# christoskokas/gtsam-vSLAM

Hardware: AMD Instinct MI355X
Metric: frames/sec (extract+match+localBA), 1500 feat stereo 752x480 (higher is better)
Workload: dtype u8/i32 (extract, match) + f64 (pose LM, local BA)

## Files before the change

gtsam-vslam_amd/csrc/ba.hip:

```cpp
#include "common.hpp"
#include "comm.hpp"
#include "dmath.hpp"
#include "ba_pool.hpp"
#include "ba_packed.hpp"
#include "ba_types.hpp"
#include "ba_order_host.hpp"
#include "ba_plan.hpp"
#include <algorithm>
#include <cmath>
#include <vector>

namespace vslam {

static_assert(BA_MAX_LEVELS == MAX_LEVELS, "BaChi::thr holds one threshold per pyramid level");
__device__ __forceinline__ int ba_slot(int sel, int c, int NB) {
    const int s = sel + 1 + c;
    return s > NB ? s - (NB + 1) : s;
}
__device__ __forceinline__ bool ba_enter(BaDev& D, int state, int c = 0) {
    const int* ci = (const int*)(D.ctl + CTL_INTS);
    if (ci[CI_STATE] != state) return false;
    D.nAct = ci[CI_NACT];
    if (c >= D.nAct) return false;
    const int sel = ci[CI_SEL], ts = ba_slot(sel, c, D.NB);
// ... 478 lines not shown
        __syncthreads();
        for (int k = 0; k < nc; k++) {
            double* dst = SpartBase + (size_t)(c0 + k) * D.spartStride + (size_t)blockIdx.x * sys;
            for (int i = threadIdx.x; i < (int)sys; i += nt) dst[i] = Sloc[(size_t)k * sys + i];
        }
    }
}

__device__ __forceinline__ double ba2_dpp_xor(double v, int which) {
    const int lo = __double2loint(v), hi = __double2hiint(v);
    int l2, h2;
    if (which == 0) { l2 = __builtin_amdgcn_update_dpp(0, lo, 0xB1, 0xF, 0xF, true); h2 = __builtin_amdgcn_update_dpp(0, hi, 0xB1, 0xF, 0xF, true); }
    else { l2 = __builtin_amdgcn_update_dpp(0, lo, 0x4E, 0xF, 0xF, true); h2 = __builtin_amdgcn_update_dpp(0, hi, 0x4E, 0xF, 0xF, true); }
    return __hiloint2double(h2, l2);
}
struct Ba2Roles {
    int hk, hq, hx, hy, hyStep; bool hOn; double hSign;
    int ws, wi;
    __device__ __forceinline__ void init(int lane) {
        hk = lane >> 2; hq = lane & 3; hOn = hk < 9;
        const int ha = hk < 3 ? 0 : (hk < 5 ? 1 : (hk == 5 ? 2 : hk - 6));
        const int hbx = hk < 3 ? hk : (hk < 5 ? hk - 2 : 2);
        hx = 14 + ha;
        hy = hk < 6 ? 14 + hbx : 0;
        hyStep = hk < 6 ? 3 : 1;
        hSign = hk < 6 ? 1.0 : -1.0;
        ws = lane / 6; wi = lane - ws * 6;
    }
};
struct Ba2Region { double* F; double* W; double* WH; double* hb; int* ffi; int* sst; int* sfi; };
__device__ __forceinline__ Ba2Region ba2_region(double* base, int maxFac, int maxSlots) {
    Ba2Region g;
    g.F = base; g.W = g.F + maxFac * 20; g.WH = g.W + maxSlots * 18; g.hb = g.WH + maxSlots * 18;
    g.ffi = (int*)(g.hb + 10); g.sst = g.ffi + maxFac; g.sfi = g.sst + maxSlots + 1;
    return g;
}
__device__ __forceinline__ void ba2_stage_h(const BaDev& D, int lp, const Ba2Region& g, const Ba2Roles& R, int lane, double* h, int& nf, int& ns) {
    const int f0 = D.lpStart[lp], s0 = D.lpSlotStart[lp];
    nf = D.lpStart[lp + 1] - f0;
    ns = D.lpSlotStart[lp + 1] - s0 - 1;
    {
        const double2* src = (const double2*)(D.facJ + (size_t)f0 * 20);
        double2* dst = (double2*)g.F;
        for (int i = lane; i < nf * 10; i += 64) dst[i] = src[i];
        for (int i = lane; i < nf; i += 64) g.ffi[i] = D.facFi[f0 + i];
        for (int i = lane; i <= ns; i += 64) { g.sst[i] = D.slotStart[s0 + i] - f0; g.sfi[i] = D.slotFi[s0 + i]; }
    }
    ba_wave_fence();
    {
        double acc = 0;
        if (R.hOn)
            for (int f = R.hq; f < nf; f += 4) {
                const double* o = g.F + f * 20;
                acc += o[R.hx] * o[R.hy] + o[R.hx + 3] * o[R.hy + R.hyStep];
            }
        acc += ba2_dpp_xor(acc, 0);
        acc += ba2_dpp_xor(acc, 1);
        if (R.hOn && R.hq == 0) g.hb[R.hk] = R.hSign * acc;
    }
    ba_wave_fence();
#pragma unroll
    for (int k = 0; k < 9; k++) h[k] = g.hb[k];
}
__device__ __forceinline__ void ba2_w_row(const Ba2Region& g, const Ba2Roles& R, double& w0, double& w1, double& w2) {
    w0 = w1 = w2 = 0;
    for (int f = g.sst[R.ws]; f < g.sst[R.ws + 1]; f++) {
        const double* o = g.F + f * 20;
        const double a0 = o[2 + R.wi], a1 = o[8 + R.wi];
        w0 += a0 * o[14] + a1 * o[17];
        w1 += a0 * o[15] + a1 * o[18];
        w2 += a0 * o[16] + a1 * o[19];
    }
}

template <bool PACKED>
__device__ __forceinline__ void ba2_blocks(double* Sloc, const double* W, const double* WH, const int* sfi, int ns, int lane, int F, int ld) {
    const int nb = ns * (ns + 1) / 2, half = lane & 1;
    for (int b0 = 0; b0 < nb; b0 += 32) {
        int b = b0 + (lane >> 1), s1 = 0;
        if (b >= nb) continue;
        while (b >= ns - s1) { b -= ns - s1; s1++; }
        const int s2 = s1 + b;
        const double* A = WH + s1 * 18 + half * 9;
        const double* B = W + s2 * 18;
        double aa[9];
#pragma unroll
        for (int q = 0; q < 9; q++) aa[q] = A[q];
        double* d0 = Sloc + (PACKED ? ba_packed_block(F, sfi[s1], sfi[s2]) * BA_PACKED_PITCH + 18 * half : (6 * sfi[s1] + 3 * half) * ld + 6 * sfi[s2]);
#pragma unroll
        for (int jh = 0; jh < 2; jh++) {
            double bb[9];
#pragma unroll
            for (int q = 0; q < 9; q++) bb[q] = B[9 * jh + q];
#pragma unroll
            for (int i = 0; i < 3; i++) {
                double* dr = d0 + i * (PACKED ? 6 : ld) + 3 * jh;
#pragma unroll
                for (int j = 0; j < 3; j++) atomicAdd(dr + j, -(aa[3 * i] * bb[3 * j] + aa[3 * i + 1] * bb[3 * j + 1] + aa[3 * i + 2] * bb[3 * j + 2]));
            }
        }
    }
}

template <bool PACKED>
__device__ __forceinline__ void ba2_schur(const BaDev* __restrict__ tab, int maxSlots, int maxFac, int layout) {
    BaDev D = *lane_entry(tab, blockIdx.z);
    extern __shared__ double sm[];
    if (!ba_enter(D, BA_TRY, blockIdx.y)) return;
    const int n = D.n, F = n / 6;
    constexpr bool packed = PACKED;
    const int ld = layout == BA2_ROWMAJOR1 ? n + 1 : n;
    const int sys = ba2_sys_doubles(n, layout);
    double* const Sloc = sm;
    double* const racc = Sloc + (packed ? ba_packed_rhs(F) : ld * n);
    const int lane = threadIdx.x & 63;
    const int unit = __builtin_amdgcn_readfirstlane(threadIdx.x >> 6), nu = blockDim.x >> 6, nt = blockDim.x;
    const Ba2Region g = ba2_region(sm + sys + (size_t)unit * ba2_stage_doubles(maxFac, maxSlots), maxFac, maxSlots);
    double* const F_ = g.F; double* const W = g.W; double* const WH = g.WH;
    int* const ffi = g.ffi; int* const sfi = g.sfi;
    const double lam = D.lambda;
    Ba2Roles R;
    R.init(lane);
    const int pf = lane / 6, pi = lane - pf * 6;
    for (int i = threadIdx.x; i < sys; i += nt) Sloc[i] = 0;
    __syncthreads();
    for (int lp = blockIdx.x * nu + unit; lp < D.Lp; lp += gridDim.x * nu) {
        double h[9];
        int nf, ns;
        ba2_stage_h(D, lp, g, R, lane, h, nf, ns);
        double Hi[9];
        ba_hll_inverse(h, lam, Hi);
        if (R.ws < ns) {
            double w0, w1, w2;
            ba2_w_row(g, R, w0, w1, w2);
            const double g0 = w0 * Hi[0] + w1 * Hi[3] + w2 * Hi[6], g1 = w0 * Hi[1] + w1 * Hi[4] + w2 * Hi[7], g2 = w0 * Hi[2] + w1 * Hi[5] + w2 * Hi[8];
            double* wr = W + R.ws * 18 + R.wi * 3;
            wr[0] = w0; wr[1] = w1; wr[2] = w2;
            double* gr = WH + R.ws * 18 + R.wi * 3;
            gr[0] = g0; gr[1] = g1; gr[2] = g2;
            atomicAdd(&racc[6 * sfi[R.ws] + R.wi], -(g0 * h[6] + g1 * h[7] + g2 * h[8]));
        }
        ba_wave_fence();
        ba2_blocks<PACKED>(Sloc, W, WH, sfi, ns, lane, F, ld);
        if (pf < 10)
            for (int fb = 0; fb < nf; fb += 10) {
                const int f = fb + pf;
                if (f >= nf) break;
                const int fi = ffi[f];
                if (fi < 0) continue;
                const double* o = F_ + f * 20;
                const double a0 = o[2 + pi], a1 = o[8 + pi];
                double* dr = Sloc + (packed ? ba_packed_block(F, fi, fi) * BA_PACKED_PITCH + 6 * pi : (6 * fi + pi) * ld + 6 * fi);
                for (int j = pi; j < 6; j++) atomicAdd(dr + j, a0 * o[2 + j] + a1 * o[8 + j]);
                atomicAdd(&racc[6 * fi + pi], -(a0 * o[0] + a1 * o[1]));
            }
        ba_wave_fence();
    }
    __syncthreads();
    const int part = ba2_part_doubles(n, layout);
    double* dst = D.Spart + (size_t)blockIdx.x * part;
    if (layout == BA2_ROWMAJOR1) {
        for (int i = threadIdx.x; i < part; i += nt) dst[i] = Sloc[i + i / n];
    } else {
        for (int i = threadIdx.x; i < part; i += nt) dst[i] = Sloc[i];
    }
}
__global__ __launch_bounds__(1024) void k_ba_schur2(const BaDev* __restrict__ tab, int maxSlots, int maxFac) { ba2_schur<true>(tab, maxSlots, maxFac, BA2_PACKED); }
__global__ __launch_bounds__(1024) void k_ba_schur2_rm(const BaDev* __restrict__ tab, int maxSlots, int maxFac, int layout) { ba2_schur<false>(tab, maxSlots, maxFac, layout); }

__global__ __launch_bounds__(512) void k_ba_back2(const BaDev* __restrict__ tab, int maxSlots, int maxFac) {
    BaDev D = *lane_entry(tab, blockIdx.z);
    extern __shared__ double sm[];
    if (!ba_enter(D, BA_TRY, 0)) return;
    const int nc = D.nAct;
    const int sel = ((const int*)(D.ctl + CTL_INTS))[CI_SEL];
    const int lane = threadIdx.x & 63;
    const int unit = __builtin_amdgcn_readfirstlane(threadIdx.x >> 6), nu = blockDim.x >> 6;
    const Ba2Region g = ba2_region(sm + (size_t)unit * ba2_stage_doubles(maxFac, maxSlots), maxFac, maxSlots);
    Ba2Roles R;
    R.init(lane);
    for (int lp = blockIdx.x * nu + unit; lp < D.Lp; lp += gridDim.x * nu) {
        double h[9];
        int nf, ns;
        ba2_stage_h(D, lp, g, R, lane, h, nf, ns);
        double w0 = 0, w1 = 0, w2 = 0;
        int kcol = 0;
        if (R.ws < ns) { ba2_w_row(g, R, w0, w1, w2); kcol = 6 * g.sfi[R.ws] + R.wi; }
        const int l = D.lpOrig[lp];
        double lamk = D.lambda;
        for (int k = 0; k < nc; k++, lamk *= 10.0) {
            const double* dPk = D.dP + (size_t)k * D.n;
            const double dp = R.ws < ns ? dPk[kcol] : 0.0;
            double t0 = w0 * dp, t1 = w1 * dp, t2 = w2 * dp;
            t0 += ba2_dpp_xor(t0, 0); t1 += ba2_dpp_xor(t1, 0); t2 += ba2_dpp_xor(t2, 0);
            t0 += ba2_dpp_xor(t0, 1); t1 += ba2_dpp_xor(t1, 1); t2 += ba2_dpp_xor(t2, 1);
#pragma unroll
            for (int d = 4; d <= 32; d <<= 1) { t0 += __shfl_xor(t0, d); t1 += __shfl_xor(t1, d); t2 += __shfl_xor(t2, d); }
            double Hi[9];
            ba_hll_inverse(h, lamk, Hi);
            if (lane < 3) {
                const double u0 = h[6] - t0, u1 = h[7] - t1, u2 = h[8] - t2;
                const double h0 = lane == 0 ? Hi[0] : (lane == 1 ? Hi[3] : Hi[6]);
                const double h1 = lane == 0 ? Hi[1] : (lane == 1 ? Hi[4] : Hi[7]);
                const double h2 = lane == 0 ? Hi[2] : (lane == 1 ? Hi[5] : Hi[8]);
                const double dl = h0 * u0 + h1 * u1 + h2 * u2;
                D.dL[(size_t)k * D.dLStride + 3 * (size_t)lp + lane] = dl;
                double* lmT = D.lmBase + (size_t)ba_slot(sel, k, D.NB) * D.lmStride;
                lmT[3 * (size_t)l + lane] = D.lmCur[3 * (size_t)l + lane] + dl;
            }
        }
        ba_wave_fence();
    }
}

__global__ __launch_bounds__(256) void k_ba_reduce(const BaDev* __restrict__ tab, int nPart, int packed) {
    BaDev D = *lane_entry(tab, blockIdx.z);
    __shared__ double sSl[8][33];
    if (!ba_enter(D, BA_TRY, blockIdx.y)) return;
    const int total = D.n * D.n + D.n, F = D.n / 6;
    const int nSum = packed ? ba_packed_doubles(F) : total;
    const int nSlots = packed ? ba_packed_reduce_slots(F) : total;
    const int e = threadIdx.x & 31, y = threadIdx.x >> 5;
    const int i = blockIdx.x * 32 + e;
    double s = 0;
    if (i < nSum) {
        const int per = (nPart + 7) / 8;
// ... 1984 lines not shown
            }
        }
    }
    BHS("chi2");
    BHS("fetch");
    if (!resultFetched) {
        VS_HIP(hipMemcpyAsync(poseOut, poseFinal, K * sizeof(DPose), hipMemcpyDeviceToHost, stream));
        if (L) VS_HIP(hipMemcpyAsync(lmOut, lmFinal, (size_t)3 * L * sizeof(double), hipMemcpyDeviceToHost, stream));
        VS_HIP(hipStreamSynchronize(stream));
    }
    ba_write_result(R, poseOut, lmOut, wrong.data(), K, L, NP);
    return VSLAM_OK;
}

static std::atomic<long long> g_bbsNs[12], g_bbsCalls{0}, g_bbsPolls{0};
static const char* g_bbsName[12] = {"check+count", "arena fill", "tables+upload", "lm pass 1", "chi2 1", "second-pass prep", "lm pass 2", "chi2 2 + fetch", "results", nullptr, nullptr, nullptr};

static BaPlanKnobs ba_plan_knobs() {
    static const bool s2Env = !(getenv("VSLAM_BA_SCHUR2") && atoi(getenv("VSLAM_BA_SCHUR2")) == 0);
    static const bool b2Env = !(getenv("VSLAM_BA_BACK2") && atoi(getenv("VSLAM_BA_BACK2")) == 0);
    BaPlanKnobs k;
    k.schur2 = s2Env; k.back2 = b2Env;
    k.sharedW = getenv("VSLAM_BA_SCHUR_SHARED") ? atoi(getenv("VSLAM_BA_SCHUR_SHARED")) != 0 : true;
    k.schurWaves = getenv("VSLAM_BA_SCHUR_WAVES_B") ? atoi(getenv("VSLAM_BA_SCHUR_WAVES_B")) : 0;
    k.lmBlocks = getenv("VSLAM_BA_LMBLOCKS") ? atoi(getenv("VSLAM_BA_LMBLOCKS")) : 0;
    k.s2Waves = getenv("VSLAM_BA_SCHUR2_WAVES") ? atoi(getenv("VSLAM_BA_SCHUR2_WAVES")) : 8;
    k.b2Waves = getenv("VSLAM_BA_BACK2_WAVES") ? atoi(getenv("VSLAM_BA_BACK2_WAVES")) : 4;
    k.s2Layout = getenv("VSLAM_BA_SCHUR2_LAYOUT") ? std::max(0, std::min((int)BA2_PACKED, atoi(getenv("VSLAM_BA_SCHUR2_LAYOUT")))) : (int)BA2_PACKED;
    return k;
}
thread_local vslam_ba_batch_plan g_baLastPlan{};

static vslam_status ba_run_batch(const vslam_ba_problem* const* Ps, vslam_ba_result* const* Rs, int N, int device) {
    g_baLastPlan = vslam_ba_batch_plan{};
    if (N <= 0 || !Ps || !Rs) return VSLAM_ERR_INVALID;
    if (N == 1) { g_baLastPlan.n_single = 1; return ba_run(Ps[0], Rs[0], device, nullptr); }
    auto bbs_t = std::chrono::steady_clock::now();
    g_bbsCalls++;
    auto BBS = [&](int k) { const auto t_ = std::chrono::steady_clock::now(); g_bbsNs[k] += std::chrono::duration_cast<std::chrono::nanoseconds>(t_ - bbs_t).count(); bbs_t = t_; };
    VS_CHECK(ba_select_device(device));
    struct BatchWs {
        hipStream_t stream = nullptr; int device = -1;
        PinnedArena arena;
// ... 123 lines not shown
        const Lane& q = lanes[i];
        nMax = std::max(nMax, q.H.n); neMax = std::max(neMax, q.H.NE);
        nfMax = std::max(nfMax, q.H.NF); npMax = std::max(npMax, q.NP);
        valMax = std::max(valMax, std::max(q.K * (int)(sizeof(DPose) / sizeof(double)), 3 * q.L));
    }
    plan_cohort();
    const vslam_ba_batch_plan& plan = g_baLastPlan;
    if (plan.status != VSLAM_OK) { set_error("local BA batch: landmark with too many views for the LDS staging"); return VSLAM_ERR_CAPACITY; }
    const int nCU = BA_NCU;
    const int obsBlocks = std::max(1, std::min((nfMax + 255) / 256, std::max(16, 2 * nCU / NL)));
    const int facBlocks = obsBlocks + std::max(neMax, 1);
    const size_t sysMax = (size_t)nMax * nMax + nMax;
    const int maxSlots = plan.max_slots, maxFac = plan.max_factors, lmBlocks = plan.schur_blocks;
    const bool useSchur2 = plan.schur_kernel == VSLAM_BA_KERNEL_SCHUR2, useBack2 = plan.back_kernel == VSLAM_BA_KERNEL_BACK2;
    const int s2Layout = ba_plan_knobs().s2Layout;
    const bool packedS = useSchur2 && s2Layout == BA2_PACKED;
    const int reduceSlots = packedS ? ba_packed_reduce_slots(nMax / 6) : (int)sysMax;
    auto part_doubles = [&](int n) { return (size_t)(useSchur2 ? ba2_part_doubles(n, s2Layout) : n * n + n); };
    const bool anyMfma64 = plan.solve_kinds & (1 << BA_SOLVE_MFMA64), anyWave = plan.solve_kinds & (1 << BA_SOLVE_WAVE),
               anyMfma = plan.solve_kinds & (1 << BA_SOLVE_MFMA);
    VS_CHECK(ba_kernel_attributes());
    size_t dBytes = 0;
    auto dtake = [&](size_t bytes) { const size_t at = dBytes; dBytes = (dBytes + std::max<size_t>(bytes, 8) + 255) & ~(size_t)255; return at; };
    struct Off { size_t flags, sedge, poseS, lmS, facJ, dP, dL, S, partial, spart, sums, Lg, wrong, outPose, outLm; };
    std::vector<Off> off(NL);
    for (int a = 0; a < NL; a++) { const Lane& q = lanes[act[a]]; off[a].flags = dtake(16 * sizeof(int)); off[a].sedge = dtake(((size_t)q.H.n * q.H.n + q.H.n) * nSlots * 8); }
    const size_t zeroBytes = dBytes;
    size_t wrongBase = 0, wrongEnd = 0, outBase = 0, outEnd = 0;
    wrongBase = dBytes;
    for (int a = 0; a < NL; a++) off[a].wrong = dtake(lanes[act[a]].NP);
    wrongEnd = dBytes;
// ... 51 lines not shown
    const BaDev* const dTab = A.dev(h_tab);
    const BaLaneAux* const dAux = A.dev(h_aux);
    VS_HIP(A.upload(stream));
    VS_HIP(hipMemsetAsync(dm, 0, zeroBytes, stream));
    const int valBlocks = std::max(1, std::min((valMax + 255) / 256, 64));
    hipLaunchKernelGGL(k_ba_init_slots_b, dim3(valBlocks, NL), dim3(256), 0, stream, dTab, dAux);

    auto step = [&](bool first) -> vslam_status {
        int t = -1;
        if (first) {
            t = g_baTimer.begin("ba_linearize");
            hipLaunchKernelGGL(k_ba_factors<0>, dim3(facBlocks, 1, NL), dim3(256), 0, stream, dTab, obsBlocks, 1, relTol, absTol);
            g_baTimer.end(t);
        }
        t = g_baTimer.begin("ba_schur");
        if (useSchur2 && s2Layout == BA2_PACKED) hipLaunchKernelGGL(k_ba_schur2, dim3(lmBlocks, NB, NL), dim3(64 * plan.schur_waves), plan.schur_lds, stream, dTab, maxSlots, maxFac);
        else if (useSchur2) hipLaunchKernelGGL(k_ba_schur2_rm, dim3(lmBlocks, NB, NL), dim3(64 * plan.schur_waves), plan.schur_lds, stream, dTab, maxSlots, maxFac, s2Layout);
        else hipLaunchKernelGGL(k_ba_schur, dim3(lmBlocks, plan.schur_shared_w ? 1 : NB, NL), dim3(64 * plan.schur_waves), plan.schur_lds, stream, dTab, maxSlots, plan.schur_shared_w);
        g_baTimer.end(t);
        t = g_baTimer.begin("ba_solve");
        hipLaunchKernelGGL(k_ba_reduce, dim3((reduceSlots + 31) / 32, NB, NL), dim3(256), 0, stream, dTab, lmBlocks, packedS ? 1 : 0);
        if (anyMfma64) hipLaunchKernelGGL(k_ba_solve_mfma64, dim3(NB, 1, NL), dim3(64), 0, stream, dTab);
        if (anyWave) hipLaunchKernelGGL(k_ba_solve_wave, dim3(NB, 1, NL), dim3(64), 0, stream, dTab);
        if (anyMfma) hipLaunchKernelGGL(k_ba_solve_mfma, dim3(NB, 1, NL), dim3(64 * BA_MFMA_NW), plan.solve_lds, stream, dTab, (double*)nullptr);
        g_baTimer.end(t);
        t = g_baTimer.begin("ba_back");
        if (useBack2) hipLaunchKernelGGL(k_ba_back2, dim3(plan.back_blocks, 1, NL), dim3(64 * plan.back_waves), plan.back_lds, stream, dTab, maxSlots, maxFac);
        else hipLaunchKernelGGL(k_ba_back, dim3(plan.back_blocks, plan.back_shared ? 1 : NB, NL), dim3(64 * plan.back_waves), plan.back_lds, stream, dTab, maxSlots, plan.back_shared);
        g_baTimer.end(t);
        t = g_baTimer.begin("ba_eval");
        hipLaunchKernelGGL(k_ba_factors<1>, dim3(facBlocks, NB, NL), dim3(256), 0, stream, dTab, obsBlocks, 1, relTol, absTol);
        g_baTimer.end(t);
        VS_HIP(hipGetLastError());
        return VSLAM_OK;
    };
    double* const b_ctl = (double*)(W.h_back + oBackCtl);
    memcpy(b_ctl, h_ctlAll, (size_t)CTL_DOUBLES * 8 * NL);
    auto lm_loop = [&](int first) -> vslam_status {
        static const int perPollEnv = getenv("VSLAM_BA_STEPS_PER_POLL") ? std::max(1, atoi(getenv("VSLAM_BA_STEPS_PER_POLL"))) : 0;
        int enq = 0, polls = 0;
        for (;;) {
            const int batch = perPollEnv ? perPollEnv : (enq == 0 ? first : 2);
// ... 82 lines not shown
        const double* lo = (const double*)(W.h_back + q.oOut + (((size_t)q.K * sizeof(DPose) + 255) & ~(size_t)255));
        ba_write_result(q.R, po, lo, W.h_back + q.oWrong, q.K, q.L, q.NP);
    }
    BBS(8);
    for (int i : redo) VS_CHECK(ba_run(Ps[i], Rs[i], device, nullptr));
    return run_singles();
}

namespace vslam {
void ba_host_profile_print() {
#ifndef VSLAM_HOST_STAMPS
    if (const long long nb = g_bbsCalls.load()) {
        fprintf(stderr, "  vslam_local_ba_batch host sections (us per cohort, %lld cohorts, %.1f polls each):", nb, (double)g_bbsPolls.load() / (double)nb);
        for (int i = 0; i < 12 && g_bbsName[i]; i++) fprintf(stderr, " %s %.1f |", g_bbsName[i], 1e-3 * (double)g_bbsNs[i].load() / (double)nb);
        fprintf(stderr, "\n");
    }
    const long long n = g_bhsCalls.load();
    if (!n) return;
    fprintf(stderr, "  vslam_local_ba host sections (us per call, %lld calls):", n);
    for (int i = 0; i < 16; i++) if (g_bhsName[i] || g_bhsNs[i].load()) fprintf(stderr, " %s %.1f |", g_bhsName[i] ? g_bhsName[i] : "other", 1e-3 * (double)g_bhsNs[i].load() / (double)n);
    fprintf(stderr, "\n");
#endif
}
}

extern "C" {

vslam_status vslam_local_ba(const vslam_ba_problem* problem, vslam_ba_result* result, int32_t device,
                            const vslam_comm* comm) {
    return ba_run(problem, result, device, comm);
// ... 211 lines not shown
```

gtsam-vslam_amd/csrc/ba_plan.hpp:

```cpp
#pragma once
#include "ba_types.hpp"
#include "ba_order_host.hpp"
#include <initializer_list>

namespace vslam {

constexpr int BA_NCU = 256;
constexpr size_t BA_LDS_SOFT = 150 * 1024;
constexpr int BA_SCHUR_LPW = 64 / BA_LPL_SCHUR, BA_BACK_LPW = 64 / BA_LPL_BACK;
inline size_t ba_stage_lds(int nw, int maxSlots) { return (size_t)nw * BA_SCHUR_LPW * 2 * maxSlots * 18 * sizeof(double) + (size_t)nw * BA_SCHUR_LPW * maxSlots * sizeof(int) + 16; }
inline size_t ba_schur_lds(int nw, int copies, size_t sysDoubles, int maxSlots) { return copies * sysDoubles * sizeof(double) + ba_stage_lds(nw, maxSlots); }
inline size_t ba_back_lds(int nw, int maxSlots) { return (size_t)nw * BA_BACK_LPW * maxSlots * 18 * sizeof(double) + (size_t)nw * BA_BACK_LPW * maxSlots * sizeof(int) + 16; }
inline int ba_schur_waves(int NB, bool allowShared, int cap, int start, size_t sysDoubles, int maxSlots, int& sharedW) {
    sharedW = 0;
    if (NB > 1 && allowShared)
        for (int nw : {16, 12, 8, 6, 4, 2})
            if (nw <= cap && ba_schur_lds(nw, NB, sysDoubles, maxSlots) <= BA_LDS_SOFT) { sharedW = 1; return nw; }
    while (start > 2 && ba_schur_lds(start, 1, sysDoubles, maxSlots) > BA_LDS_SOFT) start /= 2;
    return start;
}
inline int ba_back_waves(int cap, int maxSlots) {
    int nw = std::min(BA_SCHUR_WAVES / BA_BACK_LPW, cap);
    while (nw > 1 && ba_back_lds(nw, maxSlots) > BA_LDS_SOFT) nw /= 2;
    return nw;
// ... 114 lines not shown
    winFirst[nWin] = (int)wgWin.size();
    const int nWg = out.nWinWg = (int)wgWin.size();
    out.nInts = (size_t)2 * nWin + (nWin + 1) + (size_t)3 * std::max(nWg, 1) + std::max(total, 1);
    std::vector<int>& pack = out.pack;
    pack.reserve(out.nInts);
    pack.insert(pack.end(), winA.begin(), winA.end()); pack.insert(pack.end(), winB.begin(), winB.end());
    pack.insert(pack.end(), winFirst.begin(), winFirst.end());
    out.oWg = pack.size();
    pack.insert(pack.end(), wgWin.begin(), wgWin.end()); pack.resize(out.oWg + std::max(nWg, 1));
    pack.insert(pack.end(), wgBegin.begin(), wgBegin.end()); pack.resize(out.oWg + 2 * (size_t)std::max(nWg, 1));
    pack.insert(pack.end(), wgEnd.begin(), wgEnd.end()); pack.resize(out.oWg + 3 * (size_t)std::max(nWg, 1));
    pack.insert(pack.end(), winLm.begin(), winLm.end());
    return out;
}

struct BaPlanKnobs { bool schur2, back2, sharedW; int s2Waves, b2Waves, schurWaves, lmBlocks, s2Layout; };
inline bool ba_batch_single(const vslam_ba_lane_shape& s, bool useMfma) {
    return s.own_rig || s.n_free_kf > BA_LDS_MAX_F || s.n_free_kf <= 0 || s.n_factors <= 0 || s.n_pairs <= 0 || (!useMfma && 6 * s.n_free_kf > BA_WAVE_N);
}
inline void ba_batch_plan(const vslam_ba_batch_shape& S, const BaPlanKnobs& kn, vslam_ba_batch_plan& p) {
    p = vslam_ba_batch_plan{};
    const int NB = std::max(1, std::min((int)BA_MAX_NB, (int)S.lookahead));
    const bool useMfma = S.solver == 0;
    p.status = VSLAM_OK; p.lookahead = NB;
    int maxSlots = 1, maxFac = 1, fMax = 0, lpMax = 0, NL = 0;
    for (int i = 0; i < S.n_lanes; i++) {
        const vslam_ba_lane_shape& s = S.lanes[i];
        if (ba_batch_single(s, useMfma)) { p.n_single++; continue; }
        NL++;
        maxSlots = std::max(maxSlots, (int)s.max_slots); maxFac = std::max(maxFac, (int)s.max_factors);
        fMax = std::max(fMax, (int)s.n_free_kf); lpMax = std::max(lpMax, (int)s.n_points);
        p.solve_kinds |= 1 << ba_solve_kind(6 * s.n_free_kf, useMfma);
    }
    p.n_batch = NL; p.f_max = fMax; p.max_slots = maxSlots; p.max_factors = maxFac; p.lp_max = lpMax;
    if (NL == 0) { p.solve_kinds = 0; return; }
    const int nCU = BA_NCU, nMax = 6 * fMax;
    const size_t sysMax = (size_t)nMax * nMax + nMax;
    int sharedW = 0;
    const int schurWaves = ba_schur_waves(NB, kn.sharedW, BA_SCHUR_WAVES, kn.schurWaves ? kn.schurWaves : BA_SCHUR_WAVES, sysMax, maxSlots, sharedW);
    const size_t schurLds = ba_schur_lds(schurWaves, sharedW ? NB : 1, sysMax, maxSlots);
    const int schurUnits = schurWaves * BA_SCHUR_LPW;
    int lmBlocks = std::max(1, std::min((lpMax + schurUnits - 1) / schurUnits, kn.lmBlocks ? kn.lmBlocks : std::max(16, 2 * nCU / NL)));
    const size_t s2StageB = (size_t)ba2_stage_doubles(maxFac, maxSlots) * sizeof(double);
    int s2Waves = std::max(2, std::min(16, kn.s2Waves));
    while (s2Waves > 2 && sysMax * sizeof(double) + s2Waves * s2StageB > 156 * 1024) s2Waves /= 2;
    const size_t s2Lds = sysMax * sizeof(double) + (size_t)s2Waves * s2StageB;
    const bool useSchur2 = kn.schur2 && fMax <= BA2_MAX_F && maxSlots <= BA2_MAX_F && s2Lds <= 156 * 1024;
    if (useSchur2) lmBlocks = std::max(1, std::min((lpMax + 2 * s2Waves - 1) / (2 * s2Waves), kn.lmBlocks ? kn.lmBlocks : std::max(4, (16 / s2Waves) * nCU / NL)));
    int b2Waves = std::max(1, std::min(8, kn.b2Waves));
    while (b2Waves > 1 && (size_t)b2Waves * s2StageB > BA_DYN_LDS_MAX) b2Waves /= 2;
    const size_t b2Lds = (size_t)b2Waves * s2StageB;
    const bool useBack2 = useSchur2 && kn.back2 && b2Lds <= BA_DYN_LDS_MAX;
    const int backWaves = ba_back_waves(64, maxSlots);
    p.schur_kernel = useSchur2 ? VSLAM_BA_KERNEL_SCHUR2 : VSLAM_BA_KERNEL_SCHUR;
    p.schur_waves = useSchur2 ? s2Waves : schurWaves;
    p.schur_shared_w = useSchur2 ? 0 : sharedW;
    p.schur_blocks = lmBlocks;
    p.schur_lds = (int)(useSchur2 ? (size_t)ba2_sys_doubles(nMax, kn.s2Layout) * sizeof(double) + (size_t)s2Waves * s2StageB : schurLds);
// ... 14 lines not shown
```

gtsam-vslam_amd/csrc/ba_types.hpp:

```cpp
#pragma once
#include "dmath.hpp"
#include "ba_packed.hpp"
#include <cstddef>
#include <cstdint>

namespace vslam {

constexpr int BA_MAX_LEVELS = 12;

struct BaEdge {
    int a, b, fa, fb;
    DPose measured;
    double r[6], Ja[36], Jb[36];
    double Haa[36], Hab[36], Hbb[36], ga[6], gb[6];
};

struct BaDev {
    int NF, Lp, F, K, NE, n;
    const int* facKf; const int* facFi; const int* facLp; const int* facLm;
    const double* facZ; const double* facIs; const uint8_t* facRight;
    double* facJ;
    const int* lpStart; const int* lpSlotStart; const int* slotStart; const int* slotFi; const int* lpOrig;
    DPose* poseCur; DPose* poseTrial; const int* fidx;
    double* lmCur; double* lmTrial;
// ... 21 lines not shown
enum { BA_LINEARIZE = 0, BA_TRY = 1, BA_DONE = 2 };
enum { BA_MAX_NB = 4, SUMS_CAND = 16, FLAG_COUNT = 1, FLAG_FAIL = 4 };

constexpr int BA_SCHUR_WAVES = 16;
constexpr int BA_LDS_MAX_F = 20;
constexpr int BA_LDS_BYTES = 160 * 1024, BA_STATIC_LDS_RESERVE = 1024, BA_DYN_LDS_MAX = BA_LDS_BYTES - BA_STATIC_LDS_RESERVE;
constexpr int BA_MAX_FREE_KF = 170;

constexpr int BA_LPL_SCHUR = 64, BA_LPL_BACK = 32;

constexpr int BA2_MAX_F = 10;
BA_PACKED_HD int ba2_stage_doubles(int maxFac, int maxSlots) {
    const int ints = maxFac + 2 * (maxSlots + 1);
    return ((maxFac * 20 + 2 * maxSlots * 18 + 10 + (ints + 1) / 2) + 1) & ~1;
}
enum { BA2_ROWMAJOR = 0, BA2_ROWMAJOR1 = 1, BA2_PACKED = 2 };
BA_PACKED_HD int ba2_sys_doubles(int n, int layout) {
    return layout == BA2_PACKED ? (ba_packed_doubles(n / 6) + 1) & ~1 : layout == BA2_ROWMAJOR1 ? n * (n + 1) + n : n * n + n;
}
BA_PACKED_HD int ba2_part_doubles(int n, int layout) {
    return layout == BA2_PACKED ? ba_packed_doubles(n / 6) : n * n + n;
}

struct BaWin {
    int TB, T, TP, tileDoubles, nWin;
    const int* winA; const int* winB;
    const int* winFirstWg;
    const int* wgWin; const int* wgBegin; const int* wgEnd;
    const int* winLm;
    double* part;
// ... 23 lines not shown
```

Baseline: 30880.

## Process two thin landmarks per wave using half-wave lanes in schur2 and back2

Restructures the schur2 and back2 kernels so that each wave can take a pair of landmarks. When both landmarks are thin (few slots and factors), each 32-lane half-wave processes one of them in its own half of the LDS staging region. The aim is to recover lanes that sit idle when a landmark touches only a few keyframes. The cost is extra templated code paths, a possibly larger staging region, and a host-side cohort heuristic that picks when pairing is on, plus optional phase statistics.

```diff
diff --git a/gtsam-vslam_amd/csrc/ba.hip b/gtsam-vslam_amd/csrc/ba.hip
--- a/gtsam-vslam_amd/csrc/ba.hip
+++ b/gtsam-vslam_amd/csrc/ba.hip
@@ -516,11 +516,13 @@
     else { l2 = __builtin_amdgcn_update_dpp(0, lo, 0x4E, 0xF, 0xF, true); h2 = __builtin_amdgcn_update_dpp(0, hi, 0x4E, 0xF, 0xF, true); }
     return __hiloint2double(h2, l2);
 }
+template <int LPL>
 struct Ba2Roles {
+    static constexpr int HQ = LPL / 16;
     int hk, hq, hx, hy, hyStep; bool hOn; double hSign;
     int ws, wi;
     __device__ __forceinline__ void init(int lane) {
-        hk = lane >> 2; hq = lane & 3; hOn = hk < 9;
+        hk = lane / HQ; hq = lane % HQ; hOn = hk < 9;
         const int ha = hk < 3 ? 0 : (hk < 5 ? 1 : (hk == 5 ? 2 : hk - 6));
         const int hbx = hk < 3 ? hk : (hk < 5 ? hk - 2 : 2);
         hx = 14 + ha;
@@ -537,34 +539,33 @@
     g.ffi = (int*)(g.hb + 10); g.sst = g.ffi + maxFac; g.sfi = g.sst + maxSlots + 1;
     return g;
 }
-__device__ __forceinline__ void ba2_stage_h(const BaDev& D, int lp, const Ba2Region& g, const Ba2Roles& R, int lane, double* h, int& nf, int& ns) {
-    const int f0 = D.lpStart[lp], s0 = D.lpSlotStart[lp];
-    nf = D.lpStart[lp + 1] - f0;
-    ns = D.lpSlotStart[lp + 1] - s0 - 1;
+template <int LPL>
+__device__ __forceinline__ void ba2_stage_h(const BaDev& D, int f0, int nf, int s0, int ns, const Ba2Region& g, const Ba2Roles<LPL>& R, int lane, double* h) {
     {
         const double2* src = (const double2*)(D.facJ + (size_t)f0 * 20);
         double2* dst = (double2*)g.F;
-        for (int i = lane; i < nf * 10; i += 64) dst[i] = src[i];
-        for (int i = lane; i < nf; i += 64) g.ffi[i] = D.facFi[f0 + i];
-        for (int i = lane; i <= ns; i += 64) { g.sst[i] = D.slotStart[s0 + i] - f0; g.sfi[i] = D.slotFi[s0 + i]; }
+        for (int i = lane; i < nf * 10; i += LPL) dst[i] = src[i];
+        for (int i = lane; i < nf; i += LPL) g.ffi[i] = D.facFi[f0 + i];
+        for (int i = lane; i <= ns; i += LPL) { g.sst[i] = D.slotStart[s0 + i] - f0; g.sfi[i] = D.slotFi[s0 + i]; }
     }
     ba_wave_fence();
     {
         double acc = 0;
         if (R.hOn)
-            for (int f = R.hq; f < nf; f += 4) {
+            for (int f = R.hq; f < nf; f += Ba2Roles<LPL>::HQ) {
                 const double* o = g.F + f * 20;
                 acc += o[R.hx] * o[R.hy] + o[R.hx + 3] * o[R.hy + R.hyStep];
             }
         acc += ba2_dpp_xor(acc, 0);
-        acc += ba2_dpp_xor(acc, 1);
+        if (LPL == 64) acc += ba2_dpp_xor(acc, 1);
         if (R.hOn && R.hq == 0) g.hb[R.hk] = R.hSign * acc;
     }
     ba_wave_fence();
 #pragma unroll
     for (int k = 0; k < 9; k++) h[k] = g.hb[k];
 }
-__device__ __forceinline__ void ba2_w_row(const Ba2Region& g, const Ba2Roles& R, double& w0, double& w1, double& w2) {
+template <int LPL>
+__device__ __forceinline__ void ba2_w_row(const Ba2Region& g, const Ba2Roles<LPL>& R, double& w0, double& w1, double& w2) {
     w0 = w1 = w2 = 0;
     for (int f = g.sst[R.ws]; f < g.sst[R.ws + 1]; f++) {
         const double* o = g.F + f * 20;
@@ -575,10 +576,10 @@
     }
 }
 
-template <bool PACKED>
+template <bool PACKED, int LPL>
 __device__ __forceinline__ void ba2_blocks(double* Sloc, const double* W, const double* WH, const int* sfi, int ns, int lane, int F, int ld) {
     const int nb = ns * (ns + 1) / 2, half = lane & 1;
-    for (int b0 = 0; b0 < nb; b0 += 32) {
+    for (int b0 = 0; b0 < (LPL == 64 ? nb : 1); b0 += LPL / 2) {
         int b = b0 + (lane >> 1), s1 = 0;
         if (b >= nb) continue;
         while (b >= ns - s1) { b -= ns - s1; s1++; }
@@ -604,8 +605,47 @@
     }
 }
 
+template <bool PACKED, int LPL>
+__device__ __forceinline__ void ba2_schur_lm(const BaDev& D, double* Sloc, double* racc, const Ba2Region& g, const Ba2Roles<LPL>& R, int lane,
+                                             int f0, int nf, int s0, int ns, int F, int ld, double lam) {
+    constexpr bool packed = PACKED;
+    constexpr int PF = LPL == 64 ? 10 : 5;
+    double* const F_ = g.F; double* const W = g.W; double* const WH = g.WH;
+    int* const ffi = g.ffi; int* const sfi = g.sfi;
+    const int pf = lane / 6, pi = lane - pf * 6;
+    double h[9];
+    ba2_stage_h<LPL>(D, f0, nf, s0, ns, g, R, lane, h);
+    double Hi[9];
+    ba_hll_inverse(h, lam, Hi);
+    if (R.ws < ns) {
+        double w0, w1, w2;
+        ba2_w_row<LPL>(g, R, w0, w1, w2);
+        const double g0 = w0 * Hi[0] + w1 * Hi[3] + w2 * Hi[6], g1 = w0 * Hi[1] + w1 * Hi[4] + w2 * Hi[7], g2 = w0 * Hi[2] + w1 * Hi[5] + w2 * Hi[8];
+        double* wr = W + R.ws * 18 + R.wi * 3;
+        wr[0] = w0; wr[1] = w1; wr[2] = w2;
+        double* gr = WH + R.ws * 18 + R.wi * 3;
+        gr[0] = g0; gr[1] = g1; gr[2] = g2;
+        atomicAdd(&racc[6 * sfi[R.ws] + R.wi], -(g0 * h[6] + g1 * h[7] + g2 * h[8]));
+    }
+    ba_wave_fence();
+    ba2_blocks<PACKED, LPL>(Sloc, W, WH, sfi, ns, lane, F, ld);
+    if (pf < PF)
+        for (int fb = 0; fb < nf; fb += PF) {
+            const int f = fb + pf;
+            if (f >= nf) break;
+            const int fi = ffi[f];
+            if (fi < 0) continue;
+            const double* o = F_ + f * 20;
+            const double a0 = o[2 + pi], a1 = o[8 + pi];
+            double* dr = Sloc + (packed ? ba_packed_block(F, fi, fi) * BA_PACKED_PITCH + 6 * pi : (6 * fi + pi) * ld + 6 * fi);
+            for (int j = pi; j < 6; j++) atomicAdd(dr + j, a0 * o[2 + j] + a1 * o[8 + j]);
+            atomicAdd(&racc[6 * fi + pi], -(a0 * o[0] + a1 * o[1]));
+        }
+    ba_wave_fence();
+}
+
 template <bool PACKED>
-__device__ __forceinline__ void ba2_schur(const BaDev* __restrict__ tab, int maxSlots, int maxFac, int layout) {
+__device__ __forceinline__ void ba2_schur(const BaDev* __restrict__ tab, int maxSlots, int maxFac, int layout, int pairs) {
     BaDev D = *lane_entry(tab, blockIdx.z);
     extern __shared__ double sm[];
     if (!ba_enter(D, BA_TRY, blockIdx.y)) return;
@@ -615,48 +655,36 @@
     const int sys = ba2_sys_doubles(n, layout);
     double* const Sloc = sm;
     double* const racc = Sloc + (packed ? ba_packed_rhs(F) : ld * n);
-    const int lane = threadIdx.x & 63;
+    const int lane = threadIdx.x & 63, hf = lane >> 5, hl = lane & 31;
     const int unit = __builtin_amdgcn_readfirstlane(threadIdx.x >> 6), nu = blockDim.x >> 6, nt = blockDim.x;
-    const Ba2Region g = ba2_region(sm + sys + (size_t)unit * ba2_stage_doubles(maxFac, maxSlots), maxFac, maxSlots);
-    double* const F_ = g.F; double* const W = g.W; double* const WH = g.WH;
-    int* const ffi = g.ffi; int* const sfi = g.sfi;
+    const int regionD = ba2_region_doubles(maxFac, maxSlots), halfD = ba2_half_doubles(regionD);
+    double* const reg = sm + sys + (size_t)unit * regionD;
+    const Ba2Region g = ba2_region(reg, maxFac, maxSlots);
     const double lam = D.lambda;
-    Ba2Roles R;
+    Ba2Roles<64> R;
     R.init(lane);
-    const int pf = lane / 6, pi = lane - pf * 6;
+    Ba2Roles<32> R2;
+    R2.init(hl);
     for (int i = threadIdx.x; i < sys; i += nt) Sloc[i] = 0;
     __syncthreads();
-    for (int lp = blockIdx.x * nu + unit; lp < D.Lp; lp += gridDim.x * nu) {
-        double h[9];
-        int nf, ns;
-        ba2_stage_h(D, lp, g, R, lane, h, nf, ns);
-        double Hi[9];
-        ba_hll_inverse(h, lam, Hi);
-        if (R.ws < ns) {
-            double w0, w1, w2;
-            ba2_w_row(g, R, w0, w1, w2);
-            const double g0 = w0 * Hi[0] + w1 * Hi[3] + w2 * Hi[6], g1 = w0 * Hi[1] + w1 * Hi[4] + w2 * Hi[7], g2 = w0 * Hi[2] + w1 * Hi[5] + w2 * Hi[8];
-            double* wr = W + R.ws * 18 + R.wi * 3;
-            wr[0] = w0; wr[1] = w1; wr[2] = w2;
-            double* gr = WH + R.ws * 18 + R.wi * 3;
-            gr[0] = g0; gr[1] = g1; gr[2] = g2;
-            atomicAdd(&racc[6 * sfi[R.ws] + R.wi], -(g0 * h[6] + g1 * h[7] + g2 * h[8]));
-        }
-        ba_wave_fence();
-        ba2_blocks<PACKED>(Sloc, W, WH, sfi, ns, lane, F, ld);
-        if (pf < 10)
-            for (int fb = 0; fb < nf; fb += 10) {
-                const int f = fb + pf;
-                if (f >= nf) break;
-                const int fi = ffi[f];
-                if (fi < 0) continue;
-                const double* o = F_ + f * 20;
-                const double a0 = o[2 + pi], a1 = o[8 + pi];
-                double* dr = Sloc + (packed ? ba_packed_block(F, fi, fi) * BA_PACKED_PITCH + 6 * pi : (6 * fi + pi) * ld + 6 * fi);
-                for (int j = pi; j < 6; j++) atomicAdd(dr + j, a0 * o[2 + j] + a1 * o[8 + j]);
-                atomicAdd(&racc[6 * fi + pi], -(a0 * o[0] + a1 * o[1]));
-            }
-        ba_wave_fence();
+    const int per = pairs ? 2 : 1;
+    for (int w = blockIdx.x * nu + unit; per * w < D.Lp; w += gridDim.x * nu) {
+        int lp = per * w;
+        const int lpEnd = min(lp + per, D.Lp);
+        if (lpEnd - lp == 2) {
+            const int fa = D.lpStart[lp], fb = D.lpStart[lp + 1], fc = D.lpStart[lp + 2];
+            const int sa = D.lpSlotStart[lp], sb = D.lpSlotStart[lp + 1], sc = D.lpSlotStart[lp + 2];
+            if (ba2_thin(fb - fa, sb - sa - 1, halfD) && ba2_thin(fc - fb, sc - sb - 1, halfD)) {
+                const int f0 = hf ? fb : fa, nf = hf ? fc - fb : fb - fa, s0 = hf ? sb : sa, ns = (hf ? sc - sb : sb - sa) - 1;
+                const Ba2Region g2 = ba2_region(reg + hf * halfD, nf, ns);
+                ba2_schur_lm<PACKED, 32>(D, Sloc, racc, g2, R2, hl, f0, nf, s0, ns, F, ld, lam);
+                continue;
+            }
+        }
+        for (; lp < lpEnd; lp++) {
+            const int f0 = D.lpStart[lp], s0 = D.lpSlotStart[lp];
+            ba2_schur_lm<PACKED, 64>(D, Sloc, racc, g, R, lane, f0, D.lpStart[lp + 1] - f0, s0, D.lpSlotStart[lp + 1] - s0 - 1, F, ld, lam);
+        }
     }
     __syncthreads();
     const int part = ba2_part_doubles(n, layout);
@@ -667,51 +695,74 @@
         for (int i = threadIdx.x; i < part; i += nt) dst[i] = Sloc[i];
     }
 }
-__global__ __launch_bounds__(1024) void k_ba_schur2(const BaDev* __restrict__ tab, int maxSlots, int maxFac) { ba2_schur<true>(tab, maxSlots, maxFac, BA2_PACKED); }
-__global__ __launch_bounds__(1024) void k_ba_schur2_rm(const BaDev* __restrict__ tab, int maxSlots, int maxFac, int layout) { ba2_schur<false>(tab, maxSlots, maxFac, layout); }
-
-__global__ __launch_bounds__(512) void k_ba_back2(const BaDev* __restrict__ tab, int maxSlots, int maxFac) {
+__global__ __launch_bounds__(1024) void k_ba_schur2(const BaDev* __restrict__ tab, int maxSlots, int maxFac, int pairs) { ba2_schur<true>(tab, maxSlots, maxFac, BA2_PACKED, pairs); }
+__global__ __launch_bounds__(1024) void k_ba_schur2_rm(const BaDev* __restrict__ tab, int maxSlots, int maxFac, int layout, int pairs) { ba2_schur<false>(tab, maxSlots, maxFac, layout, pairs); }
+
+template <int LPL>
+__device__ __forceinline__ void ba2_back_lm(const BaDev& D, const Ba2Region& g, const Ba2Roles<LPL>& R, int lane, int lp, int f0, int nf, int s0, int ns, int nc, int sel) {
+    double h[9];
+    ba2_stage_h<LPL>(D, f0, nf, s0, ns, g, R, lane, h);
+    double w0 = 0, w1 = 0, w2 = 0;
+    int kcol = 0;
+    if (R.ws < ns) { ba2_w_row<LPL>(g, R, w0, w1, w2); kcol = 6 * g.sfi[R.ws] + R.wi; }
+    const int l = D.lpOrig[lp];
+    double lamk = D.lambda;
+    for (int k = 0; k < nc; k++, lamk *= 10.0) {
+        const double* dPk = D.dP + (size_t)k * D.n;
+        const double dp = R.ws < ns ? dPk[kcol] : 0.0;
+        double t0 = w0 * dp, t1 = w1 * dp, t2 = w2 * dp;
+        t0 += ba2_dpp_xor(t0, 0); t1 += ba2_dpp_xor(t1, 0); t2 += ba2_dpp_xor(t2, 0);
+        t0 += ba2_dpp_xor(t0, 1); t1 += ba2_dpp_xor(t1, 1); t2 += ba2_dpp_xor(t2, 1);
+#pragma unroll
+        for (int d = 4; d <= LPL / 2; d <<= 1) { t0 += __shfl_xor(t0, d); t1 += __shfl_xor(t1, d); t2 += __shfl_xor(t2, d); }
+        double Hi[9];
+        ba_hll_inverse(h, lamk, Hi);
+        if (lane < 3) {
+            const double u0 = h[6] - t0, u1 = h[7] - t1, u2 = h[8] - t2;
+            const double h0 = lane == 0 ? Hi[0] : (lane == 1 ? Hi[3] : Hi[6]);
+            const double h1 = lane == 0 ? Hi[1] : (lane == 1 ? Hi[4] : Hi[7]);
+            const double h2 = lane == 0 ? Hi[2] : (lane == 1 ? Hi[5] : Hi[8]);
+            const double dl = h0 * u0 + h1 * u1 + h2 * u2;
+            D.dL[(size_t)k * D.dLStride + 3 * (size_t)lp + lane] = dl;
+            double* lmT = D.lmBase + (size_t)ba_slot(sel, k, D.NB) * D.lmStride;
+            lmT[3 * (size_t)l + lane] = D.lmCur[3 * (size_t)l + lane] + dl;
+        }
+    }
+    ba_wave_fence();
+}
+__global__ __launch_bounds__(512) void k_ba_back2(const BaDev* __restrict__ tab, int maxSlots, int maxFac, int pairs) {
     BaDev D = *lane_entry(tab, blockIdx.z);
     extern __shared__ double sm[];
     if (!ba_enter(D, BA_TRY, 0)) return;
     const int nc = D.nAct;
     const int sel = ((const int*)(D.ctl + CTL_INTS))[CI_SEL];
-    const int lane = threadIdx.x & 63;
+    const int lane = threadIdx.x & 63, hf = lane >> 5, hl = lane & 31;
     const int unit = __builtin_amdgcn_readfirstlane(threadIdx.x >> 6), nu = blockDim.x >> 6;
-    const Ba2Region g = ba2_region(sm + (size_t)unit * ba2_stage_doubles(maxFac, maxSlots), maxFac, maxSlots);
-    Ba2Roles R;
+    const int regionD = ba2_region_doubles(maxFac, maxSlots), halfD = ba2_half_doubles(regionD);
+    double* const reg = sm + (size_t)unit * regionD;
+    const Ba2Region g = ba2_region(reg, maxFac, maxSlots);
+    Ba2Roles<64> R;
     R.init(lane);
-    for (int lp = blockIdx.x * nu + unit; lp < D.Lp; lp += gridDim.x * nu) {
-        double h[9];
-        int nf, ns;
-        ba2_stage_h(D, lp, g, R, lane, h, nf, ns);
-        double w0 = 0, w1 = 0, w2 = 0;
-        int kcol = 0;
-        if (R.ws < ns) { ba2_w_row(g, R, w0, w1, w2); kcol = 6 * g.sfi[R.ws] + R.wi; }
-        const int l = D.lpOrig[lp];
-        double lamk = D.lambda;
-        for (int k = 0; k < nc; k++, lamk *= 10.0) {
-            const double* dPk = D.dP + (size_t)k * D.n;
-            const double dp = R.ws < ns ? dPk[kcol] : 0.0;
-            double t0 = w0 * dp, t1 = w1 * dp, t2 = w2 * dp;
-            t0 += ba2_dpp_xor(t0, 0); t1 += ba2_dpp_xor(t1, 0); t2 += ba2_dpp_xor(t2, 0);
-            t0 += ba2_dpp_xor(t0, 1); t1 += ba2_dpp_xor(t1, 1); t2 += ba2_dpp_xor(t2, 1);
-#pragma unroll
-            for (int d = 4; d <= 32; d <<= 1) { t0 += __shfl_xor(t0, d); t1 += __shfl_xor(t1, d); t2 += __shfl_xor(t2, d); }
-            double Hi[9];
-            ba_hll_inverse(h, lamk, Hi);
-            if (lane < 3) {
-                const double u0 = h[6] - t0, u1 = h[7] - t1, u2 = h[8] - t2;
-                const double h0 = lane == 0 ? Hi[0] : (lane == 1 ? Hi[3] : Hi[6]);
-                const double h1 = lane == 0 ? Hi[1] : (lane == 1 ? Hi[4] : Hi[7]);
-                const double h2 = lane == 0 ? Hi[2] : (lane == 1 ? Hi[5] : Hi[8]);
-                const double dl = h0 * u0 + h1 * u1 + h2 * u2;
-                D.dL[(size_t)k * D.dLStride + 3 * (size_t)lp + lane] = dl;
-                double* lmT = D.lmBase + (size_t)ba_slot(sel, k, D.NB) * D.lmStride;
-                lmT[3 * (size_t)l + lane] = D.lmCur[3 * (size_t)l + lane] + dl;
-            }
-        }
-        ba_wave_fence();
+    Ba2Roles<32> R2;
+    R2.init(hl);
+    const int per = pairs ? 2 : 1;
+    for (int w = blockIdx.x * nu + unit; per * w < D.Lp; w += gridDim.x * nu) {
+        int lp = per * w;
+        const int lpEnd = min(lp + per, D.Lp);
+        if (lpEnd - lp == 2) {
+            const int fa = D.lpStart[lp], fb = D.lpStart[lp + 1], fc = D.lpStart[lp + 2];
+            const int sa = D.lpSlotStart[lp], sb = D.lpSlotStart[lp + 1], sc = D.lpSlotStart[lp + 2];
+            if (ba2_thin(fb - fa, sb - sa - 1, halfD) && ba2_thin(fc - fb, sc - sb - 1, halfD)) {
+                const int f0 = hf ? fb : fa, nf = hf ? fc - fb : fb - fa, s0 = hf ? sb : sa, ns = (hf ? sc - sb : sb - sa) - 1;
+                const Ba2Region g2 = ba2_region(reg + hf * halfD, nf, ns);
+                ba2_back_lm<32>(D, g2, R2, hl, lp + hf, f0, nf, s0, ns, nc, sel);
+                continue;
+            }
+        }
+        for (; lp < lpEnd; lp++) {
+            const int f0 = D.lpStart[lp], s0 = D.lpSlotStart[lp];
+            ba2_back_lm<64>(D, g, R, lane, lp, f0, D.lpStart[lp + 1] - f0, s0, D.lpSlotStart[lp + 1] - s0 - 1, nc, sel);
+        }
     }
 }
 
@@ -2726,6 +2777,8 @@
 }
 
 static std::atomic<long long> g_bbsNs[12], g_bbsCalls{0}, g_bbsPolls{0};
+static std::atomic<long long> g_bbsLm{0}, g_bbsPairs{0}, g_bbsThin{0}, g_bbsFacSum{0}, g_bbsSlotSum{0}, g_bbsS2{0};
+static std::atomic<int> g_bbsFacMax{0}, g_bbsSlotMax{0};
 static const char* g_bbsName[12] = {"check+count", "arena fill", "tables+upload", "lm pass 1", "chi2 1", "second-pass prep", "lm pass 2", "chi2 2 + fetch", "results", nullptr, nullptr, nullptr};
 
 static BaPlanKnobs ba_plan_knobs() {
@@ -2739,6 +2792,7 @@
     k.s2Waves = getenv("VSLAM_BA_SCHUR2_WAVES") ? atoi(getenv("VSLAM_BA_SCHUR2_WAVES")) : 8;
     k.b2Waves = getenv("VSLAM_BA_BACK2_WAVES") ? atoi(getenv("VSLAM_BA_BACK2_WAVES")) : 4;
     k.s2Layout = getenv("VSLAM_BA_SCHUR2_LAYOUT") ? std::max(0, std::min((int)BA2_PACKED, atoi(getenv("VSLAM_BA_SCHUR2_LAYOUT")))) : (int)BA2_PACKED;
+    k.s2Pairs = getenv("VSLAM_BA_SCHUR2_PAIRS") ? std::max(0, std::min(2, atoi(getenv("VSLAM_BA_SCHUR2_PAIRS")))) : 1;
     return k;
 }
 thread_local vslam_ba_batch_plan g_baLastPlan{};
@@ -2892,7 +2946,27 @@
     const int maxSlots = plan.max_slots, maxFac = plan.max_factors, lmBlocks = plan.schur_blocks;
     const bool useSchur2 = plan.schur_kernel == VSLAM_BA_KERNEL_SCHUR2, useBack2 = plan.back_kernel == VSLAM_BA_KERNEL_BACK2;
     const int s2Layout = ba_plan_knobs().s2Layout;
+    long long cohFac = 0, cohLm = 0;
+    for (int i : act) { cohFac += lanes[i].H.NF; cohLm += lanes[i].H.Lp; }
+    const int pairsKnob = ba_plan_knobs().s2Pairs;
+    const int s2Pairs = pairsKnob == 2 || (pairsKnob == 1 && cohFac <= (long long)BA2_PAIRS_MAX_FAC * cohLm) ? 1 : 0;
     const bool packedS = useSchur2 && s2Layout == BA2_PACKED;
+    static const bool phaseStats = getenv("VSLAM_BATCH_PHASES") != nullptr;
+    if (phaseStats && useSchur2) {
+        const int halfD = ba2_half_doubles(ba2_region_doubles(maxFac, maxSlots));
+        long long lm = 0, pairs = 0, thin = 0;
+        for (int i : act) {
+            const BaPassHost& H = lanes[i].H;
+            lm += H.Lp; pairs += H.Lp / 2;
+            auto thin_lm = [&](int lp) { return ba2_thin(H.h_lpStart[lp + 1] - H.h_lpStart[lp], H.h_lpSlotStart[lp + 1] - H.h_lpSlotStart[lp] - 1, halfD); };
+            for (int lp = 0; lp + 1 < H.Lp; lp += 2) thin += thin_lm(lp) && thin_lm(lp + 1);
+        }
+        g_bbsS2++; g_bbsLm += lm; g_bbsPairs += pairs; g_bbsThin += thin; g_bbsFacSum += maxFac; g_bbsSlotSum += maxSlots;
+        int m = g_bbsFacMax.load();
+        while (maxFac > m && !g_bbsFacMax.compare_exchange_weak(m, maxFac)) {}
+        m = g_bbsSlotMax.load();
+        while (maxSlots > m && !g_bbsSlotMax.compare_exchange_weak(m, maxSlots)) {}
+    }
     const int reduceSlots = packedS ? ba_packed_reduce_slots(nMax / 6) : (int)sysMax;
     auto part_doubles = [&](int n) { return (size_t)(useSchur2 ? ba2_part_doubles(n, s2Layout) : n * n + n); };
     const bool anyMfma64 = plan.solve_kinds & (1 << BA_SOLVE_MFMA64), anyWave = plan.solve_kinds & (1 << BA_SOLVE_WAVE),
@@ -2974,8 +3048,8 @@
             g_baTimer.end(t);
         }
         t = g_baTimer.begin("ba_schur");
-        if (useSchur2 && s2Layout == BA2_PACKED) hipLaunchKernelGGL(k_ba_schur2, dim3(lmBlocks, NB, NL), dim3(64 * plan.schur_waves), plan.schur_lds, stream, dTab, maxSlots, maxFac);
-        else if (useSchur2) hipLaunchKernelGGL(k_ba_schur2_rm, dim3(lmBlocks, NB, NL), dim3(64 * plan.schur_waves), plan.schur_lds, stream, dTab, maxSlots, maxFac, s2Layout);
+        if (useSchur2 && s2Layout == BA2_PACKED) hipLaunchKernelGGL(k_ba_schur2, dim3(lmBlocks, NB, NL), dim3(64 * plan.schur_waves), plan.schur_lds, stream, dTab, maxSlots, maxFac, s2Pairs);
+        else if (useSchur2) hipLaunchKernelGGL(k_ba_schur2_rm, dim3(lmBlocks, NB, NL), dim3(64 * plan.schur_waves), plan.schur_lds, stream, dTab, maxSlots, maxFac, s2Layout, s2Pairs);
         else hipLaunchKernelGGL(k_ba_schur, dim3(lmBlocks, plan.schur_shared_w ? 1 : NB, NL), dim3(64 * plan.schur_waves), plan.schur_lds, stream, dTab, maxSlots, plan.schur_shared_w);
         g_baTimer.end(t);
         t = g_baTimer.begin("ba_solve");
@@ -2985,7 +3059,7 @@
         if (anyMfma) hipLaunchKernelGGL(k_ba_solve_mfma, dim3(NB, 1, NL), dim3(64 * BA_MFMA_NW), plan.solve_lds, stream, dTab, (double*)nullptr);
         g_baTimer.end(t);
         t = g_baTimer.begin("ba_back");
-        if (useBack2) hipLaunchKernelGGL(k_ba_back2, dim3(plan.back_blocks, 1, NL), dim3(64 * plan.back_waves), plan.back_lds, stream, dTab, maxSlots, maxFac);
+        if (useBack2) hipLaunchKernelGGL(k_ba_back2, dim3(plan.back_blocks, 1, NL), dim3(64 * plan.back_waves), plan.back_lds, stream, dTab, maxSlots, maxFac, s2Pairs);
         else hipLaunchKernelGGL(k_ba_back, dim3(plan.back_blocks, plan.back_shared ? 1 : NB, NL), dim3(64 * plan.back_waves), plan.back_lds, stream, dTab, maxSlots, plan.back_shared);
         g_baTimer.end(t);
         t = g_baTimer.begin("ba_eval");
@@ -3098,6 +3172,11 @@
         fprintf(stderr, "  vslam_local_ba_batch host sections (us per cohort, %lld cohorts, %.1f polls each):", nb, (double)g_bbsPolls.load() / (double)nb);
         for (int i = 0; i < 12 && g_bbsName[i]; i++) fprintf(stderr, " %s %.1f |", g_bbsName[i], 1e-3 * (double)g_bbsNs[i].load() / (double)nb);
         fprintf(stderr, "\n");
+        if (const long long c2 = g_bbsS2.load())
+            fprintf(stderr, "  k_ba_schur2 cohorts (%lld): %.1f landmarks each, %.1f pairs of which %.1f thin (%.1f %% of the landmarks on the paired path) | (maxFac, maxSlots) mean (%.1f, %.1f) max (%d, %d)\n",
+                    c2, (double)g_bbsLm.load() / (double)c2, (double)g_bbsPairs.load() / (double)c2, (double)g_bbsThin.load() / (double)c2,
+                    200.0 * (double)g_bbsThin.load() / (double)std::max(1LL, g_bbsLm.load()), (double)g_bbsFacSum.load() / (double)c2, (double)g_bbsSlotSum.load() / (double)c2,
+                    g_bbsFacMax.load(), g_bbsSlotMax.load());
     }
     const long long n = g_bhsCalls.load();
     if (!n) return;
diff --git a/gtsam-vslam_amd/csrc/ba_plan.hpp b/gtsam-vslam_amd/csrc/ba_plan.hpp
--- a/gtsam-vslam_amd/csrc/ba_plan.hpp
+++ b/gtsam-vslam_amd/csrc/ba_plan.hpp
@@ -152,7 +152,7 @@
     return out;
 }
 
-struct BaPlanKnobs { bool schur2, back2, sharedW; int s2Waves, b2Waves, schurWaves, lmBlocks, s2Layout; };
+struct BaPlanKnobs { bool schur2, back2, sharedW; int s2Waves, b2Waves, schurWaves, lmBlocks, s2Layout, s2Pairs; };
 inline bool ba_batch_single(const vslam_ba_lane_shape& s, bool useMfma) {
     return s.own_rig || s.n_free_kf > BA_LDS_MAX_F || s.n_free_kf <= 0 || s.n_factors <= 0 || s.n_pairs <= 0 || (!useMfma && 6 * s.n_free_kf > BA_WAVE_N);
 }
@@ -179,7 +179,7 @@
     const size_t schurLds = ba_schur_lds(schurWaves, sharedW ? NB : 1, sysMax, maxSlots);
     const int schurUnits = schurWaves * BA_SCHUR_LPW;
     int lmBlocks = std::max(1, std::min((lpMax + schurUnits - 1) / schurUnits, kn.lmBlocks ? kn.lmBlocks : std::max(16, 2 * nCU / NL)));
-    const size_t s2StageB = (size_t)ba2_stage_doubles(maxFac, maxSlots) * sizeof(double);
+    const size_t s2StageB = (size_t)ba2_region_doubles(maxFac, maxSlots) * sizeof(double);
     int s2Waves = std::max(2, std::min(16, kn.s2Waves));
     while (s2Waves > 2 && sysMax * sizeof(double) + s2Waves * s2StageB > 156 * 1024) s2Waves /= 2;
     const size_t s2Lds = sysMax * sizeof(double) + (size_t)s2Waves * s2StageB;
diff --git a/gtsam-vslam_amd/csrc/ba_types.hpp b/gtsam-vslam_amd/csrc/ba_types.hpp
--- a/gtsam-vslam_amd/csrc/ba_types.hpp
+++ b/gtsam-vslam_amd/csrc/ba_types.hpp
@@ -59,6 +59,15 @@
     const int ints = maxFac + 2 * (maxSlots + 1);
     return ((maxFac * 20 + 2 * maxSlots * 18 + 10 + (ints + 1) / 2) + 1) & ~1;
 }
+constexpr int BA2_THIN_SLOTS = 5, BA2_THIN_FAC = 10;
+constexpr int BA2_PAIRS_MAX_FAC = 8;
+BA_PACKED_HD int ba2_region_doubles(int maxFac, int maxSlots) {
+    const int one = ba2_stage_doubles(maxFac, maxSlots);
+    const int two = 2 * ba2_stage_doubles(maxFac < BA2_THIN_FAC ? maxFac : BA2_THIN_FAC, maxSlots < BA2_THIN_SLOTS ? maxSlots : BA2_THIN_SLOTS);
+    return one > two ? one : two;
+}
+BA_PACKED_HD int ba2_half_doubles(int region) { return (region / 2) & ~1; }
+BA_PACKED_HD bool ba2_thin(int nf, int ns, int half) { return ns <= BA2_THIN_SLOTS && ba2_stage_doubles(nf, ns) <= half; }
 enum { BA2_ROWMAJOR = 0, BA2_ROWMAJOR1 = 1, BA2_PACKED = 2 };
 BA_PACKED_HD int ba2_sys_doubles(int n, int layout) {
     return layout == BA2_PACKED ? (ba_packed_doubles(n / 6) + 1) & ~1 : layout == BA2_ROWMAJOR1 ? n * (n + 1) + n : n * n + n;
```

Measured after the change: 30860, median of 2. No clear change (-0.1%).
